# LLNL/ppo_and_friends

Hardware: AMD Instinct MI355X
Metric: env_steps_per_sec (higher is better)
Workload: dtype f32; 1 GPU; C2 CartPole-v1 MLP (4->128x3->2 actor, ->1 critic), envs_per_proc=4096, ts_per_rollout=128, fixed-length synthetic trajectories, batch_size=256, epochs_per_iter=10; parallelism=dp1, hip_graphs=True

## Files before the change

### ppo_and_friends_amd/csrc/ppo_update_dev.hpp

```cpp
#pragma once
#include "action_heads.hpp"
#include <cstddef>
#include <cstring>

namespace ppoaf {

struct WsDev {
    float* hbuf[2];
    float* dbuf[2];
    float* outpart[2];
    float* xbuf[2];
    int W;
    int xcc[2];
    int Bp;
};

struct UpdateDev {
    NetDev net[2];
    const float* params; float* grads; float* exp_avg; float* exp_avg_sq; float* slabs;
    long bucket_total;
    int64_t* step_counts; const float* lr; double* norm_scratch;
    float beta1, beta2, adam_eps, grad_scale, max_norm; int head_kind;
    const float* obs; const float* critic_obs; const void* raw_actions;
    const float* adv; const float* old_lp; const float* rtg; float* values;
    const int64_t* perm; const int32_t* row_map; long n_rows;
    int64_t* cursor; long B, batch_stride, mb_offset, cursor_advance;
    int normalize_values, n_ranks;
    float* vn_mean; float* vn_var; double* vn_count; const double* vn_records;
    const double* adv_records;
    int normalize_adv, use_huber, pregathered;
    float surr_clip, entropy_weight, kl_loss_weight, huber_delta, min_std;
    float* loss_partials; double* totals;
    int n_wg;
    int confine;
    int split;
    WsDev sp;
    int n_slices; int slices[8];
};

inline long ws_seg_off(const NetDev& n) {
    const long szW0 = ((long)n.H * n.in_dim + 3) & ~3L;
    return n.depth == 0 ? 0 : szW0 + n.H + (long)(n.depth - 1) * ((long)n.H * n.H + n.H);
}
inline long ws_seg_len(const NetDev& n) { return n.size - ws_seg_off(n); }

inline int split_wgrad_jobs(const NetDev& n) {
    const int t = n.H / 16, t2 = (t + 1) / 2, p0 = ((n.in_dim + 15) / 16 + 1) / 2;
    return (n.depth - 1) * t * t2 + t * p0 + 1;
}
inline int split_wgrad_per_xcd(const UpdateDev& u) { return (split_wgrad_jobs(u.net[0]) + split_wgrad_jobs(u.net[1]) + 7) / 8; }
inline int split_wgrad_blocks(const UpdateDev& u) { return 8 * split_wgrad_per_xcd(u); }

inline size_t ws_layout(const UpdateDev& u, WsDev* ws, char* base) {
    const long Bp = (u.B + 63) & ~63L;
    size_t off = 0;
    auto take = [&](size_t floats) { const size_t o = off; off += (floats * 4 + 255) & ~(size_t)255; return o; };
    for (int w = 0; w < 2; ++w) {
        const NetDev& n = u.net[w];
        const size_t plane = (size_t)n.depth * Bp * n.H;
        const size_t oh = take(plane), od = take(plane), oo = take((size_t)((u.B + 15) / 16) * ws_seg_len(n));
        const size_t ox = take((size_t)Bp * 64);
        if (ws) {
            ws->hbuf[w] = reinterpret_cast<float*>(base + oh);
            ws->dbuf[w] = reinterpret_cast<float*>(base + od);
            ws->outpart[w] = reinterpret_cast<float*>(base + oo);
            ws->xbuf[w] = reinterpret_cast<float*>(base + ox);
        }
    }
    if (ws) ws->Bp = (int)Bp;
    return off;
}

constexpr int kPairHeaderBytes = 256;
constexpr int kPairRecBytes = 16 * 1024;
constexpr int kPairMaxTiles = 32;
constexpr long long kPairWaitTicks = 200000000LL;

struct PairDev {
    unsigned char* base;
    long net_off[2];
};

inline bool pair_eligible(const NetDev& n) { return n.H == 256 && n.depth >= 2 && n.depth <= 4; }
inline int pair_phases(const NetDev& n) { return 2 * n.depth - 3; }
inline size_t pair_region_offset(const UpdateDev& u) {
    UpdateDev f = u;
    if (u.batch_stride > f.B) f.B = u.batch_stride;
    return ws_layout(f, nullptr, nullptr);
}
inline size_t pair_region_layout(const UpdateDev& u, PairDev* p, char* region) {
    size_t off = kPairHeaderBytes;
    for (int w = 0; w < 2; ++w) {
        const bool on = pair_eligible(u.net[w]);
        if (p) p->net_off[w] = on ? (long)off : 0;
        if (on) off += (size_t)pair_phases(u.net[w]) * kPairMaxTiles * 2 * kPairRecBytes;
    }
    if (p) p->base = reinterpret_cast<unsigned char*>(region);
    return off;
}

constexpr int kWgradThreads = 256;

__device__ __forceinline__ void ppo_update_bookkeeping_totals(const UpdateDev& u) {
    const int lane = threadIdx.x;
    float p0 = 0.f, p2 = 0.f, p3 = 0.f, p4 = 0.f, p7 = 0.f;
    for (int g = lane; g < u.n_wg; g += 64) {
        const float* a = u.loss_partials + (long)g * 8;
        const float* cc = u.loss_partials + ((long)u.n_wg + g) * 8;
        p0 += a[0]; p3 += a[3]; p4 += a[4]; p7 += a[7]; p2 += cc[2];
    }
    p0 = wave_sum(p0); p2 = wave_sum(p2); p3 = wave_sum(p3); p4 = wave_sum(p4); p7 = wave_sum(p7);
    if (lane == 0) {
        const float n = (float)u.B;
        const float surr = p0 / n, ent = p3 / n, kl = p4 / n, crit = p2 / n;
        float total = surr;
        if (u.entropy_weight != 0.0f) total -= u.entropy_weight * ent;
        if (u.kl_loss_weight > 0.0f) total += u.kl_loss_weight * kl;
        u.totals[0] += (double)surr; u.totals[1] += (double)total; u.totals[2] += (double)crit;
        u.totals[3] += (double)ent; u.totals[4] += (double)kl;
        u.totals[5] += (double)u.loss_partials[5]; u.totals[6] += (double)u.loss_partials[6];
        u.totals[7] += p7 > 0.f ? 1.0 : 0.0;
        u.totals[8] += 1.0;
    }
}
__device__ __forceinline__ void ppo_update_bookkeeping_steps(const UpdateDev& u) {
    const int lane = threadIdx.x;
    if (lane < 2) {
        const int w = lane;
        const int64_t t = u.step_counts[w] + 1;
        u.step_counts[w] = t;
        u.norm_scratch[2 + 2 * w] = 1.0 - pow((double)u.beta1, (double)t);
        u.norm_scratch[3 + 2 * w] = sqrt(1.0 - pow((double)u.beta2, (double)t));
    }
}

__device__ __forceinline__ void ppo_update_bookkeeping_split(const UpdateDev& u) {
    if (threadIdx.x >= 64) return;
    ppo_update_bookkeeping_totals(u);
    ppo_update_bookkeeping_steps(u);
}

int make_update_dev(const ppoaf_ppo_update_args_t* a, UpdateDev& u);

inline ppoaf_ppo_update_args_t copy_update_args(const ppoaf_ppo_update_args_t* args) {
    ppoaf_ppo_update_args_t a;
    std::memset(&a, 0, sizeof(a));
    std::memcpy(&a, args, offsetof(ppoaf_ppo_update_args_t, n_action_slices));
    if (args->head_kind == PPOAF_HEAD_MULTI_CATEGORICAL) {
        a.n_action_slices = args->n_action_slices;
        std::memcpy(a.action_slices, args->action_slices, sizeof(a.action_slices));
    }
    return a;
}

__device__ __forceinline__ unsigned hw_xcc_id() {
    unsigned v;
    asm volatile("s_getreg_b32 %0, hwreg(HW_REG_XCC_ID)" : "=s"(v));
    return v & 0xfu;
}

template <bool NT, typename U>
__device__ __forceinline__ void ppo_head_loss(const U& u, const int which, const int g, const int out_dim,
                                              const float* __restrict__ log_std_p, const int* sRow,
                                              const float* sRowF, const float* sMisc, float* sActF, float* sOut,
                                              float* sDOut, const int lane, const long B) {
    const int s = lane;
    const int row = s < kRows ? sRow[s] : -1;
    const bool live = row >= 0;
    const float inv_B = 1.0f / (float)B;
    float part[8] = {0, 0, 0, 0, 0, 0, 0, 0};
    if (which == 0) {
        float logp = 0.f, ent = 0.f;
        float av = 0.f, lpo = 0.f;
        if (live) {
            av = sRowF[s]; lpo = sRowF[16 + s];
            if (u.normalize_adv) av = (av - sMisc[0]) / (sMisc[1] + 1e-8f);
        }
        if (u.head_kind == PPOAF_HEAD_CATEGORICAL) {
            const int s4 = lane >> 2, q = lane & 3;
            const bool live4 = sRow[s4] >= 0;
            float av4 = 0.f, lpo4 = 0.f;
            if (live4) {
                av4 = sRowF[s4]; lpo4 = sRowF[16 + s4];
                if (u.normalize_adv) av4 = (av4 - sMisc[0]) / (sMisc[1] + 1e-8f);
            }
            auto rsum = [](float v) { return group4_sum(v); };
            auto rmax = [](float v) { return group4_max(v); };
            const int k0 = q, k1 = q + 4;
            const bool v0 = k0 < out_dim, v1 = k1 < out_dim;
            const float z0 = v0 ? sOut[s4 * kMaxOut + k0] : -INFINITY, z1 = v1 ? sOut[s4 * kMaxOut + k1] : -INFINITY;
            const float m = rmax(fmaxf(z0, z1));
            float p0 = v0 ? expf(z0 - m) : 0.f, p1 = v1 ? expf(z1 - m) : 0.f;
            const float inv = 1.0f / rsum(p0 + p1);
            p0 *= inv; p1 *= inv;
            const float s2 = rsum(p0 + p1);
            int a = reinterpret_cast<const int*>(sActF)[s4 * 8];
            a = a < 0 ? 0 : (a >= out_dim ? out_dim - 1 : a);
            const float n0 = p0 / s2, n1 = p1 / s2;
            const float l0 = v0 ? logf(clamp_prob_u(n0)) : 0.f, l1 = v1 ? logf(clamp_prob_u(n1)) : 0.f;
            const float ent4 = -rsum((v0 ? n0 * l0 : 0.f) + (v1 ? n1 * l1 : 0.f));
            const float logp4 = rsum((k0 == a ? l0 : 0.f) + (k1 == a ? l1 : 0.f));
            const float ratio = expf(logp4 - lpo4);
            const float bad4 = (isnan(ratio) || isinf(ratio)) ? 1.f : 0.f;
            const float lo = 1.0f - u.surr_clip, hi = 1.0f + u.surr_clip;
            const float surr1 = ratio * av4, surr2 = fminf(fmaxf(ratio, lo), hi) * av4;
            float glp;
            if (surr1 <= surr2) glp = -av4 * ratio;
            else glp = (ratio >= lo && ratio <= hi) ? -av4 * ratio : 0.f;
            glp *= inv_B;
            const float gH = (u.entropy_weight != 0.0f) ? -u.entropy_weight * inv_B : 0.f;
            auto gk_of = [&](bool valid, int k, float nk, float lg) {
                if (!valid) return 0.f;
                const float ck = clamp_prob_u(nk);
                const float in_range = (nk >= FLT_EPSILON && nk <= 1.0f - FLT_EPSILON) ? 1.f : 0.f;
                float gk = gH * (-lg - nk * in_range / ck);
                if (k == a) gk += glp * in_range / ck;
                return gk;
            };
            float g0 = gk_of(v0, k0, n0, l0), g1 = gk_of(v1, k1, n1, l1);
            const float dot = rsum(g0 * n0 + g1 * n1);
            g0 = (g0 - dot) / s2; g1 = (g1 - dot) / s2;
            const float dot2 = rsum(g0 * p0 + g1 * p1);
            if (live4) {
                if (k0 < 8) sDOut[s4 * kMaxOut + k0] = p0 * (g0 - dot2);
                sDOut[s4 * kMaxOut + k1] = p1 * (g1 - dot2);
            } else {
                sDOut[s4 * kMaxOut + k0] = 0.f; sDOut[s4 * kMaxOut + k1] = 0.f;
                if (q == 0) for (int k2 = 8; k2 < kMaxOut; ++k2) sDOut[s4 * kMaxOut + k2] = 0.f;
            }
            const int src = (lane & 15) * 4;
            const float r_surr = __shfl(-fminf(surr1, surr2), src, 64), r_ent = __shfl(ent4, src, 64);
            const float r_kl = __shfl(lpo4 - logp4, src, 64), r_bad = __shfl(bad4, src, 64);
            if (live) { part[0] = r_surr; part[3] = r_ent; part[4] = r_kl; part[7] = r_bad; }
        } else if (u.head_kind >= PPOAF_HEAD_MULTI_CATEGORICAL) {
            if (live) {
                float z[8], dz[8];
#pragma unroll
                for (int k = 0; k < 8; ++k) z[k] = k < out_dim ? sOut[s * kMaxOut + k] : 0.f;
                const bool mcat = u.head_kind == PPOAF_HEAD_MULTI_CATEGORICAL;
                const float* x = sActF + s * 8;
                float p[8], sm[8];
                unsigned first = 0u, pick = 0u;
                if (mcat) {
                    first = mcat_starts(u.n_slices, u.slices);
                    mcat_probs(z, first, out_dim, p, sm);
                    pick = mcat_pick(reinterpret_cast<const int*>(x), u.n_slices, u.slices);
                    logp = mcat_logp(p, sm, pick);
                } else {
                    logp = bern_logp(z, x, out_dim);
                }
                const float ratio = expf(logp - lpo);
                if (isnan(ratio) || isinf(ratio)) part[7] = 1.f;
                const float lo = 1.0f - u.surr_clip, hi = 1.0f + u.surr_clip;
                const float surr1 = ratio * av, surr2 = fminf(fmaxf(ratio, lo), hi) * av;
                float glp;
                if (surr1 <= surr2) glp = -av * ratio;
                else glp = (ratio >= lo && ratio <= hi) ? -av * ratio : 0.f;
                glp *= inv_B;
                const float gH = (u.entropy_weight != 0.0f) ? -u.entropy_weight * inv_B : 0.f;
                ent = mcat ? mcat_entropy_grad(p, sm, first, pick, out_dim, glp, gH, dz)
                           : bern_entropy_grad(z, x, out_dim, glp, gH, dz);
                part[0] = -fminf(surr1, surr2);
                part[3] = ent;
                part[4] = lpo - logp;
#pragma unroll
                for (int k = 0; k < 8; ++k) sDOut[s * kMaxOut + k] = dz[k];
            } else if (s < kRows) {
                for (int k = 0; k < kMaxOut; ++k) sDOut[s * kMaxOut + k] = 0.f;
            }
        } else if (live) {
            const float* log_std = log_std_p;
            const float* x = sActF + s * 8;
            float lp = 0.f, slog = 0.f;
            ent = 0.f;
            for (int d = 0; d < out_dim; ++d) {
                const float sd = fmaxf(softplus_u(ld1<NT>(log_std + d)), u.min_std);
                const float mu = sOut[s * kMaxOut + d];
                const float zz = x[d] - mu;
                const float l0 = -logf(sd) - 0.91893853320467274178f;
                float l = -(zz * zz) / (2.0f * sd * sd) + l0;
                l = fminf(fmaxf(l, -100.f), 100.f);
                lp += l;
                const float th = tanhf(x[d]);
                slog += logf(fmaxf(1.0f - th * th, 1e-6f));
                const float thm = tanhf(mu);
                ent += logf(fmaxf(1.0f - thm * thm, 1e-6f)) - fminf(fmaxf(l0, -100.f), 100.f);
            }
            logp = lp - slog;
            const float ratio = expf(logp - lpo);
            if (isnan(ratio) || isinf(ratio)) part[7] = 1.f;
            const float lo = 1.0f - u.surr_clip, hi = 1.0f + u.surr_clip;
            const float surr1 = ratio * av, surr2 = fminf(fmaxf(ratio, lo), hi) * av;
            part[0] = -fminf(surr1, surr2);
            part[3] = ent;
            part[4] = lpo - logp;
            float glp;
            if (surr1 <= surr2) glp = -av * ratio;
            else glp = (ratio >= lo && ratio <= hi) ? -av * ratio : 0.f;
            glp *= inv_B;
            const float gH = (u.entropy_weight != 0.0f) ? -u.entropy_weight * inv_B : 0.f;
            for (int d = 0; d < out_dim; ++d) {
                const float ls = ld1<NT>(log_std + d);
                const float sp = softplus_u(ls), sd = fmaxf(sp, u.min_std);
                const float mu = sOut[s * kMaxOut + d];
                const float zz = x[d] - mu;
                const float l0 = -logf(sd) - 0.91893853320467274178f;
                const float l = -(zz * zz) / (2.0f * sd * sd) + l0;
                const float pass = (l >= -100.f && l <= 100.f) ? 1.f : 0.f;
                const float pass0 = (l0 >= -100.f && l0 <= 100.f) ? 1.f : 0.f;
                const float thm = tanhf(mu);
                const float pass_t = (1.0f - thm * thm >= 1e-6f) ? 1.f : 0.f;
                sDOut[s * kMaxOut + d] = glp * pass * zz / (sd * sd) - gH * pass_t * 2.0f * thm;
                if (d == 0) for (int k2 = out_dim; k2 < 8; ++k2) sDOut[s * kMaxOut + k2] = 0.f;
                const float dmax = sp > u.min_std ? 1.f : (sp == u.min_std ? 0.5f : 0.f);
                const float dsp = ls > 20.f ? 1.f : 1.0f / (1.0f + expf(-ls));
                sOut[s * kMaxOut + 8 + d] = (glp * pass * (zz * zz / (sd * sd * sd) - 1.0f / sd) + gH * pass0 / sd) * dmax * dsp;
            }
        } else if (s < kRows) {
            for (int k = 0; k < kMaxOut; ++k) sDOut[s * kMaxOut + k] = 0.f;
            if (u.head_kind == PPOAF_HEAD_GAUSSIAN)
                for (int d = 0; d < 8; ++d) sOut[s * kMaxOut + 8 + d] = 0.f;
        }
    } else {
        if (live) {
            const float v = sOut[s * kMaxOut];
            float rt = sRowF[32 + s];
            if (u.normalize_values) rt = (rt - sMisc[2]) / sqrtf(sMisc[3] + 1e-8f);
            const float diff = v - rt;
            float l, dl;
            if (u.use_huber) {
                const float ad = fabsf(diff);
                if (ad < u.huber_delta) { l = 0.5f * diff * diff; dl = diff; }
                else { l = u.huber_delta * (ad - 0.5f * u.huber_delta); dl = diff > 0.f ? u.huber_delta : -u.huber_delta; }
            } else { l = diff * diff; dl = 2.0f * diff; }
            part[2] = l;
            sDOut[s * kMaxOut] = dl * inv_B;
            for (int k2 = 1; k2 < 8; ++k2) sDOut[s * kMaxOut + k2] = 0.f;
            u.values[row] = v;
        } else if (s < kRows) {
            for (int k2 = 0; k2 < 8; ++k2) sDOut[s * kMaxOut + k2] = 0.f;
        }
    }
#pragma unroll
    for (int k = 0; k < 8; ++k) {
        float v = (lane < kRows) ? part[k] : 0.f;
        v = group16_sum(v);
        part[k] = v;
    }
    if (lane == 0) {
        if (which == 0 && g == 0) { part[5] = sMisc[0]; part[6] = sMisc[1]; }
        float* lp = u.loss_partials + ((long)which * u.n_wg + g) * 8;
#pragma unroll
        for (int k = 0; k < 8; ++k) lp[k] = part[k];
    }
}

}
```

### ppo_and_friends_amd/csrc/ppo_update_rowtile.hpp

```cpp
#pragma once
#include "ppo_update_dev.hpp"

namespace ppoaf {

extern __shared__ __attribute__((aligned(16))) unsigned char ppo_update_smem[];

#ifdef PPOAF_STAMPS
#ifndef PPOAF_STAMP_BLOCK
#define PPOAF_STAMP_BLOCK 0
#endif
static __device__ unsigned long long g_ppo_update_stamps[2][16];
#define PPOAF_STAMP(k)                                                                   \
    do {                                                                                 \
        if (blockIdx.x == PPOAF_STAMP_BLOCK && threadIdx.x == 0) {                       \
            unsigned long long t_;                                                       \
            asm volatile("s_memtime %0\n\ts_waitcnt lgkmcnt(0)" : "=s"(t_)::"memory");    \
            g_ppo_update_stamps[0][k] = t_;                                              \
        }                                                                                \
    } while (0)
#else
#define PPOAF_STAMP(k) do {} while (0)
#endif



template <int HT, bool NT>
__device__ __forceinline__ void load_fwd_set(const float* __restrict__ W, int n0, int lane, float4 (&fr)[HT]) {
    if constexpr (NT) load_fwd_frags<HT, true>(W, n0, lane, fr);
    else load_fwd_lines_buf<HT>(W, n0, lane, fr);
}
template <int HT, bool NT>
__device__ __forceinline__ f32x4 mfma_fwd_set(const float* __restrict__ A, int HS, int lane, const float4 (&fr)[HT], float init,
                                              float* __restrict__ scratch) {
    if constexpr (NT) return mfma_rows_x_frags<HT>(A, HS, lane, fr, init);
    else return mfma_rows_x_lines<HT>(A, HS, lane, fr, init, scratch);
}

__device__ __forceinline__ int rowtile_request_args(const UpdateDev& u, int b) {
    const NetDev& a = u.net[0];
    const NetDev& c = u.net[1];
    asm("" : "+s"(b)
        : "s"(a.in_dim), "s"(a.H), "s"(a.depth), "s"(a.out_dim), "s"(a.act), "s"((&a.act)[1]), "s"(a.offset), "s"(a.size), "s"(a.log_std_off),
          "s"(c.in_dim), "s"(c.H), "s"(c.depth), "s"(c.out_dim), "s"(c.act), "s"((&c.act)[1]), "s"(c.offset), "s"(c.size), "s"(c.log_std_off),
          "s"(u.params), "s"(u.norm_scratch), "s"(u.head_kind),
          "s"(u.obs), "s"(u.critic_obs), "s"(u.raw_actions), "s"(u.adv), "s"(u.old_lp), "s"(u.rtg), "s"(u.values), "s"(u.perm),
          "s"(u.row_map), "s"(u.n_rows), "s"(u.cursor), "s"(u.B), "s"(u.batch_stride), "s"(u.mb_offset), "s"(u.cursor_advance),
          "s"(u.normalize_values), "s"(u.n_ranks), "s"(u.vn_mean), "s"(u.vn_var), "s"(u.vn_count), "s"(u.vn_records),
          "s"(u.adv_records), "s"(u.normalize_adv), "s"(u.use_huber), "s"(u.pregathered), "s"(u.surr_clip),
          "s"(u.n_wg), "s"(u.confine));
    const long cur = u.cursor[0];
    asm("" : "+s"(b)
        : "s"(cur), "s"(u.entropy_weight), "s"(u.kl_loss_weight), "s"(u.huber_delta), "s"(u.min_std), "s"(u.loss_partials),
          "s"(u.sp.hbuf[0]), "s"(u.sp.hbuf[1]), "s"(u.sp.dbuf[0]), "s"(u.sp.dbuf[1]), "s"(u.sp.outpart[0]), "s"(u.sp.outpart[1]),
          "s"(u.sp.xbuf[0]), "s"(u.sp.xbuf[1]), "s"(u.sp.W), "s"(u.sp.xcc[0]), "s"(u.sp.xcc[1]), "s"(u.sp.Bp), "s"(u.n_slices),
          "s"(u.slices[0]), "s"(u.slices[1]), "s"(u.slices[2]), "s"(u.slices[3]), "s"(u.slices[4]), "s"(u.slices[5]),
          "s"(u.slices[6]), "s"(u.slices[7]));
    return b;
}

template <int HT, bool SPLIT, bool TABLES>
__device__ __forceinline__ void ppo_update_fwd_bwd_body_as(const UpdateDev& u, const int which, const int g) {
    constexpr bool NT = false;
    constexpr long mb_extra = 0;
    constexpr int H = 16 * HT, HS = H + 4;
    int tid_ = threadIdx.x;
    if (NT) {
        asm volatile("" : "+v"(tid_));
        __builtin_assume(tid_ >= 0 && tid_ < kThreadsU);
    }
    const int tid = tid_, lane = tid & 63, wave = NT ? __builtin_amdgcn_readfirstlane(tid >> 6) : (tid >> 6);
    const auto& nd = u.net[which];
    const int in_dim = nd.in_dim, depth = nd.depth, out_dim = nd.out_dim, act = nd.act;
    const int NT0 = (in_dim + 15) >> 4;
    const int INP = 16 * NT0 + 4;
    const float* P = u.params + nd.offset;
    const long B = u.B;
    const long mb = u.cursor[0] + u.mb_offset + mb_extra;
    const long base = mb * u.batch_stride;
    const long szW0 = ((long)H * in_dim + 3) & ~3L;
    auto offW = [&](int l) -> long { return l == 0 ? 0 : szW0 + H + (long)(l - 1) * (H * H + H); };
    auto offB = [&](int l) -> long {
        return l == 0 ? szW0 : offW(l) + (l < depth ? (long)H * H : (((long)out_dim * H + 3) & ~3L));
    };
    float* slab = SPLIT ? u.sp.outpart[which] + (long)g * (nd.size - offW(depth)) - offW(depth)
                        : u.slabs + (long)g * u.bucket_total + nd.offset;
    auto publish_rows = [&](const float* src, float* panel) {
        float* dst = panel + (long)g * kRows * H;
        for (int i = tid; i < kRows * (H / 4); i += kThreadsU) {
            const int r = i / (H / 4), c4 = i - r * (H / 4);
            *reinterpret_cast<float4*>(dst + (long)r * H + 4 * c4) = *reinterpret_cast<const float4*>(src + r * HS + 4 * c4);
        }
    };
    const long sp_plane = SPLIT ? (long)u.sp.Bp * H : 0;

    PPOAF_STAMP(0);
    int zl = 0;
    if (NT) asm volatile("" : "+s"(zl));
    float* smem = reinterpret_cast<float*>(ppo_update_smem + zl);
    int* sRow = reinterpret_cast<int*>(smem);
    float* sMisc = smem + 16;
    float* sRowF = smem + 32;
    float* sActF = smem + 80;
    float* sBias = smem + 208;
    float* sWout = sBias + (depth + 1) * H;
    float* sX = sWout + 8 * H;
    float* sH = sX + kRows * INP;
    float* sD0 = sH + (long)depth * kRows * HS;
    float* sD1 = sD0 + kRows * HS;
    float* sOut = sD1 + kRows * HS;
    float* sDOut = sOut + kRows * kMaxOut;
    float* sScr = sDOut + kRows * kMaxOut + wave * 2 * kLineSlot;

    if (!NT && g == 0 && which == 0 && tid == 0) { u.norm_scratch[0] = 0.0; u.norm_scratch[1] = 0.0; }

    const bool has_tile = HT >= kNW || wave < HT;
    static_assert(!TABLES || HT <= kNW, "deep prefetch: one output tile per wave");
    const bool deep = TABLES || (depth == 3 && HT <= kNW);
    float4 fr[HT], fr2[HT];
    const bool l0_pre = in_dim <= 16 && HT <= kNW && has_tile;
    float l0w[4] = {0.f, 0.f, 0.f, 0.f};
    float l2_touch = 0.f;
    constexpr int kCopyRegs = 4;
    float bias_reg[kCopyRegs], wout_reg[kCopyRegs];
    const int n_bias = (depth + 1) * H, n_wout = out_dim * H;
    const bool copy_fits = n_bias <= kCopyRegs * kThreadsU && n_wout <= kCopyRegs * kThreadsU;
    auto request_weights = [&]() {
        if (NT && deep && has_tile) {
            load_fwd_set<HT, NT>(P + offW(1), wave * 16, lane, fr);
            load_fwd_set<HT, NT>(P + offW(2), wave * 16, lane, fr2);
        }
        if (l0_pre) {
            const float* w = P + offW(0) + (long)(wave * 16 + (lane & 15)) * in_dim;
#pragma unroll
            for (int j = 0; j < 4; ++j) { const int k = 4 * j + (lane >> 4); if (k < in_dim) l0w[j] = ld1<NT>(w + k); }
        }
#ifndef PPOAF_L2_TOUCH_MAX_HT
#define PPOAF_L2_TOUCH_MAX_HT 8
#endif
        if (!deep && !NT && HT <= PPOAF_L2_TOUCH_MAX_HT) for (long i = (long)tid * 32; i < nd.size; i += (long)kThreadsU * 32) l2_touch += P[i];
        if (copy_fits) {
#pragma unroll
            for (int r = 0; r < kCopyRegs; ++r) {
                const int i = tid + r * kThreadsU;
                bias_reg[r] = 0.f; wout_reg[r] = 0.f;
                if (i < n_bias) { const int l = i / H, j = i - l * H; if (l < depth || j < out_dim) bias_reg[r] = ld1<NT>(P + offB(l) + j); }
                if (i < n_wout) wout_reg[r] = ld1<NT>(P + offW(depth) + i);
            }
        }
    };
    auto request_hidden_sets = [&]() {
        if (!NT && deep && has_tile) {
            load_fwd_set<HT, NT>(P + offW(1), wave * 16, lane, fr);
            load_fwd_set<HT, NT>(P + offW(2), wave * 16, lane, fr2);
        }
    };
    const float* x_src = which == 0 ? u.obs : u.critic_obs;
    const bool x_pre = !NT && (TABLES || u.pregathered) && kRows * in_dim <= 2 * kThreadsU;
    float xr[2] = {0.f, 0.f};
    if (x_pre) {
#pragma unroll
        for (int q = 0; q < 2; ++q) {
            const int idx = tid + q * kThreadsU;
            if (idx < kRows * in_dim && (long)g * kRows + idx / in_dim < B) xr[q] = x_src[(base + (long)g * kRows) * in_dim + idx];
        }
    }
    if constexpr (TABLES) asm volatile("; ppoaf_rowtile_tables_prologue");
    if (!NT) request_weights();

    constexpr int kActRegs = 8;
    constexpr int kVnPre = 2;
    const bool row_lane = tid < kRows && (long)g * kRows + tid < B;
    static_assert(!TABLES || !NT, "per-epoch tables: separate launches only");
    constexpr bool early = TABLES;
    const int n_act = which != 0 ? 0 : u.head_kind == PPOAF_HEAD_CATEGORICAL ? 1
                    : u.head_kind == PPOAF_HEAD_MULTI_CATEGORICAL ? u.n_slices : out_dim;
    long perm_v = -1;
    float av = 0.f, lpo = 0.f, rt = 0.f;
    int act_bits[kActRegs];
#pragma unroll
    for (int j = 0; j < kActRegs; ++j) act_bits[j] = 0;
    auto request_row_scalars = [&](const long di) {
        if (which == 0) {
            av = u.adv[di]; lpo = u.old_lp[di];
            if (u.head_kind == PPOAF_HEAD_CATEGORICAL) {
                act_bits[0] = (int)reinterpret_cast<const int64_t*>(u.raw_actions)[di];
            } else if (u.head_kind == PPOAF_HEAD_MULTI_CATEGORICAL) {
#pragma unroll
                for (int j = 0; j < kActRegs; ++j)
                    if (j < n_act) act_bits[j] = (int)reinterpret_cast<const int64_t*>(u.raw_actions)[(long)di * u.n_slices + j];
            } else {
#pragma unroll
                for (int d = 0; d < kActRegs; ++d)
                    if (d < n_act) act_bits[d] = __float_as_int(reinterpret_cast<const float*>(u.raw_actions)[(long)di * out_dim + d]);
            }
        } else {
            rt = u.rtg[di];
        }
    };
    if (row_lane) {
        const long s = (long)g * kRows + tid;
        perm_v = u.perm[base + s];
        if (early) request_row_scalars(base + s);
    }
    const bool stat_lane = tid == 64;
    double adv_rec[3] = {0.0, 0.0, 0.0}, vn_rec[kVnPre][3];
    float vn_m = 0.f, vn_v = 0.f;
    double vn_cnt = 0.0;
#pragma unroll
    for (int r = 0; r < kVnPre; ++r) { vn_rec[r][0] = 0.0; vn_rec[r][1] = 0.0; vn_rec[r][2] = 0.0; }
    if (stat_lane) {
        if (which == 0) {
            if (u.normalize_adv) {
                const double* rec = u.adv_records + mb * 3;
                adv_rec[0] = rec[0]; adv_rec[1] = rec[1]; adv_rec[2] = rec[2];
            }
        } else {
            const int slot = (int)(mb & 1);
            vn_m = ld1<NT>(u.vn_mean + slot); vn_v = ld1<NT>(u.vn_var + slot);
            vn_cnt = ld1<NT>(u.vn_count + slot);
            if (u.normalize_values) {
#pragma unroll
                for (int r = 0; r < kVnPre; ++r) {
                    if (r < u.n_ranks) {
                        const double* rec = u.vn_records + (mb * u.n_ranks + r) * 3;
                        vn_rec[r][0] = rec[0]; vn_rec[r][1] = rec[1]; vn_rec[r][2] = rec[2];
                    }
                }
            }
        }
    }
    double vn_n = 0.0, vn_bm = 0.0, vn_M2 = 0.0;
    auto vn_merge = [&](const double nb, const double mean, const double m2) {
        if (nb <= 0.0) return;
        const double d = mean - vn_bm, nn = vn_n + nb;
        vn_bm += d * (nb / nn);
        vn_M2 += m2 + d * d * vn_n * nb / nn;
        vn_n = nn;
    };
    if (stat_lane && which != 0 && u.normalize_values && u.n_ranks > kVnPre) {
#pragma unroll
        for (int r = 0; r < kVnPre; ++r) vn_merge(vn_rec[r][0], vn_rec[r][1], vn_rec[r][2]);
        for (int r = kVnPre; r < u.n_ranks; ++r) {
            const double* rec = u.vn_records + (mb * u.n_ranks + r) * 3;
            vn_merge(rec[0], rec[1], rec[2]);
        }
    }
    if (!NT) request_hidden_sets();

    if (tid < kRows) {
        auto store_row = [&](const int row, const bool have) {
            if (have) {
#pragma unroll
                for (int j = 0; j < kActRegs; ++j)
                    if (j < n_act) reinterpret_cast<int*>(sActF)[tid * 8 + j] = act_bits[j];
            }
            sRow[tid] = row;
            sRowF[tid] = av; sRowF[16 + tid] = lpo; sRowF[32 + tid] = rt;
        };
        if constexpr (TABLES) {
            int row = -1;
            if (row_lane && perm_v >= 0 && perm_v < u.n_rows) row = (int)perm_v;
            store_row(row, row_lane);
        } else {
            int row = -1;
            long di = -1;
            if (row_lane) {
                const long p = perm_v;
                if (p >= 0 && p < u.n_rows) row = u.row_map ? u.row_map[p] : (int)p;
                di = u.pregathered ? base + (long)g * kRows + tid : row;
            }
            if (di >= 0 && !early) request_row_scalars(di);
            store_row(row, di >= 0);
        }
    }

    if (stat_lane) {
        if (which == 0) {
            float mean_f = 0.f, std_f = 1.f;
            if (u.normalize_adv) {
                mean_f = (float)adv_rec[1];
                std_f = (float)sqrt(adv_rec[2] / (adv_rec[0] - 1.0));
            }
            sMisc[0] = mean_f; sMisc[1] = std_f;
        } else {
            const int slot = (int)(mb & 1);
            float m = vn_m, v = vn_v;
            double cnt = vn_cnt;
            if (u.normalize_values) {
                if (u.n_ranks <= kVnPre) {
#pragma unroll
                    for (int r = 0; r < kVnPre; ++r)
                        if (r < u.n_ranks) vn_merge(vn_rec[r][0], vn_rec[r][1], vn_rec[r][2]);
                }
                const double n = vn_n, bm = vn_bm, M2 = vn_M2;
                if (n > 0.0) {
                    const float batch_mean = (float)bm, batch_var = (float)(M2 / n);
                    const float delta = batch_mean - m;
                    const double new_count = cnt + n;
                    const float new_mean = (float)((double)m + (double)delta * (n / new_count));
                    const double m_2 = (double)v * cnt + (double)batch_var * n +
                                       (double)(delta * delta) * cnt * n / (cnt + n);
                    m = new_mean; v = (float)(m_2 / (cnt + n)); cnt = new_count;
                }
            }
            sMisc[2] = m; sMisc[3] = v;
            if (g == 0) { u.vn_mean[slot ^ 1] = m; u.vn_var[slot ^ 1] = v; u.vn_count[slot ^ 1] = cnt; }
        }
    }
    if (copy_fits) {
#pragma unroll
        for (int r = 0; r < kCopyRegs; ++r) {
            const int i = tid + r * kThreadsU;
            if (i < n_bias) sBias[i] = bias_reg[r];
            if (i < n_wout) sWout[i] = wout_reg[r];
        }
    } else {
        for (int l = 0; l <= depth; ++l) {
            const int n = (l == depth) ? out_dim : H;
            const float* bb = P + offB(l);
            for (int i = tid; i < n; i += kThreadsU) sBias[l * H + i] = ld1<NT>(bb + i);
        }
        for (int i = tid; i < out_dim * H; i += kThreadsU) sWout[i] = ld1<NT>(P + offW(depth) + i);
    }
    for (int i = tid; i < kRows * INP; i += kThreadsU) sX[i] = 0.f;
    __syncthreads();
    PPOAF_STAMP(1);

    if (x_pre) {
#pragma unroll
        for (int q = 0; q < 2; ++q) {
            const int idx = tid + q * kThreadsU;
            const int s = idx / in_dim, i = idx - s * in_dim;
            if (idx < kRows * in_dim && sRow[s] >= 0) sX[s * INP + i] = xr[q];
        }
    } else {
        const float* src = x_src;
        for (int idx = tid; idx < kRows * in_dim; idx += kThreadsU) {
            const int s = idx / in_dim, i = idx - s * in_dim;
            const int row = sRow[s];
            const long di = (TABLES || u.pregathered) ? base + (long)g * kRows + s : row;
            if (row >= 0) sX[s * INP + i] = src[di * in_dim + i];
        }
    }
    if (!deep && depth > 1 && has_tile) load_fwd_set<HT, NT>(P + offW(1), wave * 16, lane, fr);
    __syncthreads();
    PPOAF_STAMP(2);
    if (SPLIT) {
        float* xb = u.sp.xbuf[which] + (long)g * kRows * 64;
        for (int i = tid; i < kRows * 64; i += kThreadsU) {
            const int r = i >> 6, c = i & 63;
            xb[i] = c < 16 * NT0 ? sX[r * INP + c] : 0.f;
        }
    }

    for (int nt = wave; nt < HT; nt += kNW) {
        const int o = nt * 16 + (lane & 15);
        const float bv = sBias[o];
        f32x4 acc = {bv, bv, bv, bv};
        const float* w = P + offW(0) + (long)o * in_dim;
        const float* arow = sX + (lane & 15) * INP;
        for (int k0 = 0; k0 < in_dim; k0 += 16) {
            float bq[4];
#pragma unroll
            for (int j = 0; j < 4; ++j) {
                const int k = k0 + 4 * j + (lane >> 4);
                bq[j] = l0_pre ? l0w[j] : (k < in_dim ? ld1<NT>(w + k) : 0.f);
            }
#pragma unroll
            for (int j = 0; j < 4; ++j)
                acc = __builtin_amdgcn_mfma_f32_16x16x4f32(arow[k0 + 4 * j + (lane >> 4)], bq[j], acc, 0, 0, 0);
        }
#pragma unroll
        for (int r = 0; r < 4; ++r) sH[(4 * (lane >> 4) + r) * HS + o] = act_fwd(acc[r], act);
    }
    __syncthreads();
    PPOAF_STAMP(3);

    for (int l = 1; l < depth; ++l) {
        const float* Hp = sH + (long)(l - 1) * kRows * HS;
        float* Hc = sH + (long)l * kRows * HS;
        if (SPLIT) publish_rows(Hp, u.sp.hbuf[which] + (long)(l - 1) * sp_plane);
        for (int nt = wave; nt < HT; nt += kNW) {
            const int o = nt * 16 + (lane & 15);
            f32x4 acc;
            if (deep) {
                if (l == 1) {
                    acc = mfma_fwd_set<HT, NT>(Hp, HS, lane, fr, sBias[l * H + o], sScr);
                    load_dgrad_frags<HT, NT>(P + offW(2), wave * 16, lane, fr);
                } else {
                    acc = mfma_fwd_set<HT, NT>(Hp, HS, lane, fr2, sBias[l * H + o], sScr);
                    load_dgrad_frags<HT, NT>(P + offW(1), wave * 16, lane, fr2);
                }
            } else {
            if (nt != wave) load_fwd_set<HT, NT>(P + offW(l), nt * 16, lane, fr);
            acc = mfma_fwd_set<HT, NT>(Hp, HS, lane, fr, sBias[l * H + o], sScr);
            if (nt + kNW >= HT) {
                if (l + 1 < depth) load_fwd_set<HT, NT>(P + offW(l + 1), wave * 16, lane, fr);
                else load_dgrad_frags<HT, NT>(P + offW(l), wave * 16, lane, fr);
            }
            }
#pragma unroll
            for (int r = 0; r < 4; ++r) Hc[(4 * (lane >> 4) + r) * HS + o] = act_fwd(acc[r], act);
            
        }
        __syncthreads();
        
    }
    PPOAF_STAMP(4);
    const float* Hlast = sH + (long)(depth - 1) * kRows * HS;

    if (tid < 256) {
        const int s = tid >> 4, part = tid & 15;
        for (int k = 0; k < out_dim; ++k) {
            float acc = 0.f;
#pragma unroll
            for (int i = 0; i < HT; ++i) acc = fmaf(Hlast[s * HS + part + 16 * i], sWout[k * H + part + 16 * i], acc);
            acc = group16_sum(acc);
            if (part == 0) sOut[s * kMaxOut + k] = acc + sBias[depth * H + k];
        }
    }
    __syncthreads();
    PPOAF_STAMP(5);

    if (wave == 0) {
        ppo_head_loss<NT>(u, which, g, out_dim, P + nd.log_std_off, sRow, sRowF, sMisc, sActF, sOut, sDOut, lane, B);
    }
    __syncthreads();
    PPOAF_STAMP(6);

    {
        if (tid < H) {
            const int i = tid;
            float h[kRows];
#pragma unroll
            for (int s = 0; s < kRows; ++s) h[s] = Hlast[s * HS + i];
            for (int k = 0; k < out_dim; ++k) {
                float d[kRows];
#pragma unroll
                for (int s = 0; s < kRows; ++s) d[s] = sDOut[s * kMaxOut + k];
                float acc = 0.f;
#pragma unroll
                for (int s = 0; s < kRows; ++s) acc = fmaf(d[s], h[s], acc);
                slab[offW(depth) + (long)k * H + i] = acc;
            }
        }
        const int out_pad = SPLIT ? ((out_dim + 3) & ~3) : out_dim;
        if (tid >= 256 && tid < 256 + out_pad) {
            const int k = tid - 256;
            float acc = 0.f;
            if (k < out_dim) {
#pragma unroll
                for (int s = 0; s < kRows; ++s) acc += sDOut[s * kMaxOut + k];
            }
            slab[offB(depth) + k] = acc;
        }
        if (which == 0 && u.head_kind == PPOAF_HEAD_GAUSSIAN && tid >= 320 && tid < 320 + out_pad) {
            const int d = tid - 320;
            float acc = 0.f;
            if (d < out_dim) {
#pragma unroll
                for (int s = 0; s < kRows; ++s) acc += sOut[s * kMaxOut + 8 + d];
            }
            slab[nd.log_std_off + d] = acc;
        }
        if (tid >= 256) {
            const int t2 = tid - 256;
            const int s = t2 >> 4, ig = t2 & 15;
            float d[8];
            const float4 d0 = *reinterpret_cast<const float4*>(sDOut + s * kMaxOut);
            const float4 d1 = *reinterpret_cast<const float4*>(sDOut + s * kMaxOut + 4);
            d[0] = d0.x; d[1] = d0.y; d[2] = d0.z; d[3] = d0.w; d[4] = d1.x; d[5] = d1.y; d[6] = d1.z; d[7] = d1.w;
            float hv[HT], acc[HT];
#pragma unroll
            for (int ii = 0; ii < HT; ++ii) { hv[ii] = Hlast[s * HS + ig + 16 * ii]; acc[ii] = 0.f; }
#pragma unroll
            for (int k = 0; k < 8; ++k) {
                if (k < out_dim) {
#pragma unroll
                    for (int ii = 0; ii < HT; ++ii) acc[ii] = fmaf(d[k], sWout[k * H + ig + 16 * ii], acc[ii]);
                }
            }
#pragma unroll
            for (int ii = 0; ii < HT; ++ii) sD0[s * HS + ig + 16 * ii] = acc[ii] * act_bwd(hv[ii], act);
        }
    }
    __syncthreads();
    PPOAF_STAMP(7);

    float* Dc = sD0;
    float* Dn = sD1;
    for (int l = depth - 1; l >= 1; --l) {
        const float* Hin = sH + (long)(l - 1) * kRows * HS;
        if (SPLIT) publish_rows(Dc, u.sp.dbuf[which] + (long)l * sp_plane);
        for (int nt = wave; nt < HT; nt += kNW) {
            f32x4 acc;
            if (deep) {
                acc = l == 2 ? mfma_rows_x_frags<HT>(Dc, HS, lane, fr, 0.f) : mfma_rows_x_frags<HT>(Dc, HS, lane, fr2, 0.f);
            } else {
            if (nt != wave) load_dgrad_frags<HT, NT>(P + offW(l), nt * 16, lane, fr);
            acc = mfma_rows_x_frags<HT>(Dc, HS, lane, fr, 0.f);
            if (nt + kNW >= HT && l - 1 >= 1) load_dgrad_frags<HT, NT>(P + offW(l - 1), wave * 16, lane, fr);
            }
#pragma unroll
            for (int r = 0; r < 4; ++r) {
                const int s = 4 * (lane >> 4) + r, i = nt * 16 + (lane & 15);
                Dn[s * HS + i] = acc[r] * act_bwd(Hin[s * HS + i], act);
            }
        }
        if (l == depth - 1) PPOAF_STAMP(10);
        if (!SPLIT) {
            for (int mt = wave; mt < HT; mt += kNW) {
                if (HT <= 8) wgrad_mtile_full<(HT <= 8 ? HT : 1)>(Dc, HS, Hin, HS, mt * 16, lane, slab + offW(l), H);
                else wgrad_mtile(Dc, HS, Hin, HS, mt * 16, HT, H, lane, slab + offW(l), H);
            }
            if (l == depth - 1) PPOAF_STAMP(11);
            for (int o = tid; o < H; o += kThreadsU) {
                float acc = 0.f;
#pragma unroll
                for (int s = 0; s < kRows; ++s) acc += Dc[s * HS + o];
                slab[offB(l) + o] = acc;
            }
        }
        if (l == depth - 1) PPOAF_STAMP(12);
        __syncthreads();
        if (l == depth - 1) PPOAF_STAMP(13);
        float* t = Dc; Dc = Dn; Dn = t;
    }
    PPOAF_STAMP(8);

    if (SPLIT) {
        publish_rows(Dc, u.sp.dbuf[which]);
    } else {
        for (int mt = wave; mt < HT; mt += kNW)
            wgrad_mtile(Dc, HS, sX, INP, mt * 16, NT0, in_dim, lane, slab + offW(0), in_dim);
        for (int o = tid; o < H; o += kThreadsU) {
            float acc = 0.f;
#pragma unroll
            for (int s = 0; s < kRows; ++s) acc += Dc[s * HS + o];
            slab[offB(0) + o] = acc;
        }
    }
    if (l2_touch == 1.2345e38f) u.loss_partials[0] = l2_touch;
    PPOAF_STAMP(9);
}

template <int HT, bool SPLIT = false>
__device__ __forceinline__ void ppo_update_fwd_bwd_body(const UpdateDev& u, const int which, const int g) {
    if constexpr (HT <= kNW) {
        if (u.net[which].depth == 3 && u.pregathered && !u.row_map) {
            ppo_update_fwd_bwd_body_as<HT, SPLIT, true>(u, which, g);
            return;
        }
    }
    ppo_update_fwd_bwd_body_as<HT, SPLIT, false>(u, which, g);
}

constexpr size_t kRowtileLineFloats = (size_t)kNW * 2 * kLineSlot;
inline size_t rowtile_lds_floats(const NetDev& n) {
    const size_t HS = n.H + 4, INP = 16 * ((n.in_dim + 15) / 16) + 4;
    return 208 + (size_t)(n.depth + 1) * n.H + 8 * (size_t)n.H + kRows * INP + (size_t)n.depth * kRows * HS + 2 * kRows * HS +
           2 * kRows * kMaxOut;
}

}
```

Before: 1.133 million env-steps/s.

## Fuse head forward, loss and dgrad per row-group and defer head weight-grad tail

In the TABLES path, each 16-lane group now computes its row's output logits, head loss and output dgrad itself, separated only by wavefront barriers, so two block-wide __syncthreads are gone. The head loss is split into a per-row function, and the loss-partial reduction, output weight-grad and bias grads move into a deferred tail. By default that tail runs inside the first hidden backward layer, overlapping with the MFMA dgrad work. The change also keeps the first two output-weight rows in registers and preloads the Hlast column for the tail threads, which raises register pressure.

After: 1.133 million env-steps/s, median of 2. No clear change (+0.0%).

```diff
diff --git a/ppo_and_friends_amd/csrc/ppo_update_dev.hpp b/ppo_and_friends_amd/csrc/ppo_update_dev.hpp
--- a/ppo_and_friends_amd/csrc/ppo_update_dev.hpp
+++ b/ppo_and_friends_amd/csrc/ppo_update_dev.hpp
@@ -159,16 +159,14 @@
     return v & 0xfu;
 }
 
-template <bool NT, typename U>
-__device__ __forceinline__ void ppo_head_loss(const U& u, const int which, const int g, const int out_dim,
-                                              const float* __restrict__ log_std_p, const int* sRow,
-                                              const float* sRowF, const float* sMisc, float* sActF, float* sOut,
-                                              float* sDOut, const int lane, const long B) {
-    const int s = lane;
-    const int row = s < kRows ? sRow[s] : -1;
+template <bool NT, typename U, typename Z>
+__device__ __forceinline__ void ppo_head_row(const U& u, const int which, const int out_dim,
+                                             const float* __restrict__ log_std_p, const int* sRow, const float* sRowF,
+                                             const float* sMisc, const float* sActF, float* sOut, float* sDOut, const int s,
+                                             const int q, const bool writer, const Z& zval, const long B, float (&part)[8]) {
+    const int row = sRow[s];
     const bool live = row >= 0;
     const float inv_B = 1.0f / (float)B;
-    float part[8] = {0, 0, 0, 0, 0, 0, 0, 0};
     if (which == 0) {
         float logp = 0.f, ent = 0.f;
         float av = 0.f, lpo = 0.f;
@@ -177,36 +175,29 @@
             if (u.normalize_adv) av = (av - sMisc[0]) / (sMisc[1] + 1e-8f);
         }
         if (u.head_kind == PPOAF_HEAD_CATEGORICAL) {
-            const int s4 = lane >> 2, q = lane & 3;
-            const bool live4 = sRow[s4] >= 0;
-            float av4 = 0.f, lpo4 = 0.f;
-            if (live4) {
-                av4 = sRowF[s4]; lpo4 = sRowF[16 + s4];
-                if (u.normalize_adv) av4 = (av4 - sMisc[0]) / (sMisc[1] + 1e-8f);
-            }
             auto rsum = [](float v) { return group4_sum(v); };
             auto rmax = [](float v) { return group4_max(v); };
             const int k0 = q, k1 = q + 4;
             const bool v0 = k0 < out_dim, v1 = k1 < out_dim;
-            const float z0 = v0 ? sOut[s4 * kMaxOut + k0] : -INFINITY, z1 = v1 ? sOut[s4 * kMaxOut + k1] : -INFINITY;
+            const float z0 = v0 ? zval(k0) : -INFINITY, z1 = v1 ? zval(k1) : -INFINITY;
             const float m = rmax(fmaxf(z0, z1));
             float p0 = v0 ? expf(z0 - m) : 0.f, p1 = v1 ? expf(z1 - m) : 0.f;
             const float inv = 1.0f / rsum(p0 + p1);
             p0 *= inv; p1 *= inv;
             const float s2 = rsum(p0 + p1);
-            int a = reinterpret_cast<const int*>(sActF)[s4 * 8];
+            int a = reinterpret_cast<const int*>(sActF)[s * 8];
             a = a < 0 ? 0 : (a >= out_dim ? out_dim - 1 : a);
             const float n0 = p0 / s2, n1 = p1 / s2;
             const float l0 = v0 ? logf(clamp_prob_u(n0)) : 0.f, l1 = v1 ? logf(clamp_prob_u(n1)) : 0.f;
             const float ent4 = -rsum((v0 ? n0 * l0 : 0.f) + (v1 ? n1 * l1 : 0.f));
             const float logp4 = rsum((k0 == a ? l0 : 0.f) + (k1 == a ? l1 : 0.f));
-            const float ratio = expf(logp4 - lpo4);
+            const float ratio = expf(logp4 - lpo);
             const float bad4 = (isnan(ratio) || isinf(ratio)) ? 1.f : 0.f;
             const float lo = 1.0f - u.surr_clip, hi = 1.0f + u.surr_clip;
-            const float surr1 = ratio * av4, surr2 = fminf(fmaxf(ratio, lo), hi) * av4;
+            const float surr1 = ratio * av, surr2 = fminf(fmaxf(ratio, lo), hi) * av;
             float glp;
-            if (surr1 <= surr2) glp = -av4 * ratio;
-            else glp = (ratio >= lo && ratio <= hi) ? -av4 * ratio : 0.f;
+            if (surr1 <= surr2) glp = -av * ratio;
+            else glp = (ratio >= lo && ratio <= hi) ? -av * ratio : 0.f;
             glp *= inv_B;
             const float gH = (u.entropy_weight != 0.0f) ? -u.entropy_weight * inv_B : 0.f;
             auto gk_of = [&](bool valid, int k, float nk, float lg) {
@@ -221,22 +212,21 @@
             const float dot = rsum(g0 * n0 + g1 * n1);
             g0 = (g0 - dot) / s2; g1 = (g1 - dot) / s2;
             const float dot2 = rsum(g0 * p0 + g1 * p1);
-            if (live4) {
-                if (k0 < 8) sDOut[s4 * kMaxOut + k0] = p0 * (g0 - dot2);
-                sDOut[s4 * kMaxOut + k1] = p1 * (g1 - dot2);
-            } else {
-                sDOut[s4 * kMaxOut + k0] = 0.f; sDOut[s4 * kMaxOut + k1] = 0.f;
-                if (q == 0) for (int k2 = 8; k2 < kMaxOut; ++k2) sDOut[s4 * kMaxOut + k2] = 0.f;
+            if (writer) {
+                if (live) {
+                    if (k0 < 8) sDOut[s * kMaxOut + k0] = p0 * (g0 - dot2);
+                    sDOut[s * kMaxOut + k1] = p1 * (g1 - dot2);
+                } else {
+                    sDOut[s * kMaxOut + k0] = 0.f; sDOut[s * kMaxOut + k1] = 0.f;
+                    if (q == 0) for (int k2 = 8; k2 < kMaxOut; ++k2) sDOut[s * kMaxOut + k2] = 0.f;
+                }
             }
-            const int src = (lane & 15) * 4;
-            const float r_surr = __shfl(-fminf(surr1, surr2), src, 64), r_ent = __shfl(ent4, src, 64);
-            const float r_kl = __shfl(lpo4 - logp4, src, 64), r_bad = __shfl(bad4, src, 64);
-            if (live) { part[0] = r_surr; part[3] = r_ent; part[4] = r_kl; part[7] = r_bad; }
+            if (live) { part[0] = -fminf(surr1, surr2); part[3] = ent4; part[4] = lpo - logp4; part[7] = bad4; }
         } else if (u.head_kind >= PPOAF_HEAD_MULTI_CATEGORICAL) {
             if (live) {
                 float z[8], dz[8];
 #pragma unroll
-                for (int k = 0; k < 8; ++k) z[k] = k < out_dim ? sOut[s * kMaxOut + k] : 0.f;
+                for (int k = 0; k < 8; ++k) z[k] = k < out_dim ? zval(k) : 0.f;
                 const bool mcat = u.head_kind == PPOAF_HEAD_MULTI_CATEGORICAL;
                 const float* x = sActF + s * 8;
                 float p[8], sm[8];
@@ -265,7 +255,7 @@
                 part[4] = lpo - logp;
 #pragma unroll
                 for (int k = 0; k < 8; ++k) sDOut[s * kMaxOut + k] = dz[k];
-            } else if (s < kRows) {
+            } else {
                 for (int k = 0; k < kMaxOut; ++k) sDOut[s * kMaxOut + k] = 0.f;
             }
         } else if (live) {
@@ -275,7 +265,7 @@
             ent = 0.f;
             for (int d = 0; d < out_dim; ++d) {
                 const float sd = fmaxf(softplus_u(ld1<NT>(log_std + d)), u.min_std);
-                const float mu = sOut[s * kMaxOut + d];
+                const float mu = zval(d);
                 const float zz = x[d] - mu;
                 const float l0 = -logf(sd) - 0.91893853320467274178f;
                 float l = -(zz * zz) / (2.0f * sd * sd) + l0;
@@ -302,7 +292,7 @@
             for (int d = 0; d < out_dim; ++d) {
                 const float ls = ld1<NT>(log_std + d);
                 const float sp = softplus_u(ls), sd = fmaxf(sp, u.min_std);
-                const float mu = sOut[s * kMaxOut + d];
+                const float mu = zval(d);
                 const float zz = x[d] - mu;
                 const float l0 = -logf(sd) - 0.91893853320467274178f;
                 const float l = -(zz * zz) / (2.0f * sd * sd) + l0;
@@ -316,14 +306,14 @@
                 const float dsp = ls > 20.f ? 1.f : 1.0f / (1.0f + expf(-ls));
                 sOut[s * kMaxOut + 8 + d] = (glp * pass * (zz * zz / (sd * sd * sd) - 1.0f / sd) + gH * pass0 / sd) * dmax * dsp;
             }
-        } else if (s < kRows) {
+        } else {
             for (int k = 0; k < kMaxOut; ++k) sDOut[s * kMaxOut + k] = 0.f;
             if (u.head_kind == PPOAF_HEAD_GAUSSIAN)
                 for (int d = 0; d < 8; ++d) sOut[s * kMaxOut + 8 + d] = 0.f;
         }
     } else {
         if (live) {
-            const float v = sOut[s * kMaxOut];
+            const float v = zval(0);
             float rt = sRowF[32 + s];
             if (u.normalize_values) rt = (rt - sMisc[2]) / sqrtf(sMisc[3] + 1e-8f);
             const float diff = v - rt;
@@ -337,10 +327,15 @@
             sDOut[s * kMaxOut] = dl * inv_B;
             for (int k2 = 1; k2 < 8; ++k2) sDOut[s * kMaxOut + k2] = 0.f;
             u.values[row] = v;
-        } else if (s < kRows) {
+        } else {
             for (int k2 = 0; k2 < 8; ++k2) sDOut[s * kMaxOut + k2] = 0.f;
         }
     }
+}
+
+template <typename U>
+__device__ __forceinline__ void ppo_head_partials(const U& u, const int which, const int g, const float* sMisc,
+                                                  const int lane, float (&part)[8]) {
 #pragma unroll
     for (int k = 0; k < 8; ++k) {
         float v = (lane < kRows) ? part[k] : 0.f;
@@ -355,4 +350,25 @@
     }
 }
 
-}
+template <bool NT, typename U>
+__device__ __forceinline__ void ppo_head_loss(const U& u, const int which, const int g, const int out_dim,
+                                              const float* __restrict__ log_std_p, const int* sRow,
+                                              const float* sRowF, const float* sMisc, float* sActF, float* sOut,
+                                              float* sDOut, const int lane, const long B) {
+    float part[8] = {0, 0, 0, 0, 0, 0, 0, 0};
+    if (which == 0 && u.head_kind == PPOAF_HEAD_CATEGORICAL) {
+        const int s4 = lane >> 2;
+        float r[8] = {0, 0, 0, 0, 0, 0, 0, 0};
+        ppo_head_row<NT>(u, which, out_dim, log_std_p, sRow, sRowF, sMisc, sActF, sOut, sDOut, s4, lane & 3, true,
+                         [&](const int k) { return sOut[s4 * kMaxOut + k]; }, B, r);
+        const int src = (lane & 15) * 4;
+        part[0] = __shfl(r[0], src, 64); part[3] = __shfl(r[3], src, 64);
+        part[4] = __shfl(r[4], src, 64); part[7] = __shfl(r[7], src, 64);
+    } else if (lane < kRows) {
+        ppo_head_row<NT>(u, which, out_dim, log_std_p, sRow, sRowF, sMisc, sActF, sOut, sDOut, lane, 0, true,
+                         [&](const int k) { return sOut[lane * kMaxOut + k]; }, B, part);
+    }
+    ppo_head_partials(u, which, g, sMisc, lane, part);
+}
+
+}
diff --git a/ppo_and_friends_amd/csrc/ppo_update_rowtile.hpp b/ppo_and_friends_amd/csrc/ppo_update_rowtile.hpp
--- a/ppo_and_friends_amd/csrc/ppo_update_rowtile.hpp
+++ b/ppo_and_friends_amd/csrc/ppo_update_rowtile.hpp
@@ -409,83 +409,204 @@
     PPOAF_STAMP(4);
     const float* Hlast = sH + (long)(depth - 1) * kRows * HS;
 
-    if (tid < 256) {
-        const int s = tid >> 4, part = tid & 15;
-        for (int k = 0; k < out_dim; ++k) {
-            float acc = 0.f;
-#pragma unroll
-            for (int i = 0; i < HT; ++i) acc = fmaf(Hlast[s * HS + part + 16 * i], sWout[k * H + part + 16 * i], acc);
-            acc = group16_sum(acc);
-            if (part == 0) sOut[s * kMaxOut + k] = acc + sBias[depth * H + k];
-        }
-    }
-    __syncthreads();
-    PPOAF_STAMP(5);
-
-    if (wave == 0) {
-        ppo_head_loss<NT>(u, which, g, out_dim, P + nd.log_std_off, sRow, sRowF, sMisc, sActF, sOut, sDOut, lane, B);
-    }
-    __syncthreads();
-    PPOAF_STAMP(6);
-
-    {
-        if (tid < H) {
-            const int i = tid;
-            float h[kRows];
-#pragma unroll
-            for (int s = 0; s < kRows; ++s) h[s] = Hlast[s * HS + i];
-            for (int k = 0; k < out_dim; ++k) {
+    const int out_pad = SPLIT ? ((out_dim + 3) & ~3) : out_dim;
+#ifndef PPOAF_HEAD_TAIL_AT
+#define PPOAF_HEAD_TAIL_AT 1
+#endif
+    constexpr int kDwThreads = kThreadsU - 256;
+    constexpr bool kPreH = TABLES && PPOAF_HEAD_TAIL_AT != 2 && kDwThreads % H == 0;
+    float hcol[kRows];
+    auto head_tail = [&]() {
+        if (wave >= 4) {
+            for (int idx = tid - 256; idx < out_dim * H; idx += kDwThreads) {
+                const int k = idx / H, i = idx - k * H;
+                if (!kPreH) {
+#pragma unroll
+                    for (int s = 0; s < kRows; ++s) hcol[s] = Hlast[s * HS + i];
+                }
                 float d[kRows];
 #pragma unroll
                 for (int s = 0; s < kRows; ++s) d[s] = sDOut[s * kMaxOut + k];
                 float acc = 0.f;
 #pragma unroll
-                for (int s = 0; s < kRows; ++s) acc = fmaf(d[s], h[s], acc);
+                for (int s = 0; s < kRows; ++s) acc = fmaf(d[s], hcol[s], acc);
                 slab[offW(depth) + (long)k * H + i] = acc;
             }
-        }
-        const int out_pad = SPLIT ? ((out_dim + 3) & ~3) : out_dim;
-        if (tid >= 256 && tid < 256 + out_pad) {
-            const int k = tid - 256;
-            float acc = 0.f;
-            if (k < out_dim) {
-#pragma unroll
-                for (int s = 0; s < kRows; ++s) acc += sDOut[s * kMaxOut + k];
-            }
-            slab[offB(depth) + k] = acc;
-        }
-        if (which == 0 && u.head_kind == PPOAF_HEAD_GAUSSIAN && tid >= 320 && tid < 320 + out_pad) {
-            const int d = tid - 320;
-            float acc = 0.f;
-            if (d < out_dim) {
-#pragma unroll
-                for (int s = 0; s < kRows; ++s) acc += sOut[s * kMaxOut + 8 + d];
-            }
-            slab[nd.log_std_off + d] = acc;
-        }
-        if (tid >= 256) {
-            const int t2 = tid - 256;
-            const int s = t2 >> 4, ig = t2 & 15;
+        } else if (wave == 0) {
+            float part[8];
+#pragma unroll
+            for (int k = 0; k < 8; ++k) part[k] = lane < kRows ? sOut[lane * kMaxOut + k] : 0.f;
+            ppo_head_partials(u, which, g, sMisc, lane, part);
+        } else if (wave == 1) {
+            if (lane < out_pad) {
+                const int k = lane;
+                float acc = 0.f;
+                if (k < out_dim) {
+#pragma unroll
+                    for (int s = 0; s < kRows; ++s) acc += sDOut[s * kMaxOut + k];
+                }
+                slab[offB(depth) + k] = acc;
+            }
+        } else if (wave == 2) {
+            if (which == 0 && u.head_kind == PPOAF_HEAD_GAUSSIAN && lane < out_pad) {
+                const int d = lane;
+                float acc = 0.f;
+                if (d < out_dim) {
+#pragma unroll
+                    for (int s = 0; s < kRows; ++s) acc += sOut[s * kMaxOut + 8 + d];
+                }
+                slab[nd.log_std_off + d] = acc;
+            }
+        }
+    };
+    if constexpr (TABLES) {
+        asm volatile("; ppoaf_rowtile_head_phase_begin");
+        if (tid < 256) {
+            const int s = tid >> 4, part = tid & 15;
+            constexpr int kKeepW = 2;
+            float hv[HT], wk[kKeepW][HT];
+#pragma unroll
+            for (int i = 0; i < HT; ++i) { hv[i] = Hlast[s * HS + part + 16 * i]; wk[0][i] = 0.f; wk[1][i] = 0.f; }
+#pragma unroll
+            for (int k = 0; k < 8; ++k) {
+                if (k < out_dim) {
+                    float w[HT];
+#pragma unroll
+                    for (int i = 0; i < HT; ++i) w[i] = sWout[k * H + part + 16 * i];
+                    float acc = 0.f;
+#pragma unroll
+                    for (int i = 0; i < HT; ++i) acc = fmaf(hv[i], w[i], acc);
+                    if (k < kKeepW) {
+#pragma unroll
+                        for (int i = 0; i < HT; ++i) wk[k < kKeepW ? k : 0][i] = w[i];
+                    }
+                    acc = group16_sum(acc);
+                    if (part == 0) sOut[s * kMaxOut + k] = acc + sBias[depth * H + k];
+                }
+            }
+            __builtin_amdgcn_fence(__ATOMIC_ACQ_REL, "wavefront");
+            __builtin_amdgcn_wave_barrier();
+            PPOAF_STAMP(5);
+            auto zval = [&](const int k) { return sOut[s * kMaxOut + k]; };
+            float pr[8] = {0, 0, 0, 0, 0, 0, 0, 0};
+            if (which == 0 && u.head_kind == PPOAF_HEAD_CATEGORICAL) {
+                ppo_head_row<NT>(u, which, out_dim, P + nd.log_std_off, sRow, sRowF, sMisc, sActF, sOut, sDOut, s, part & 3,
+                                 part < 4, zval, B, pr);
+            } else if (part == 0) {
+                ppo_head_row<NT>(u, which, out_dim, P + nd.log_std_off, sRow, sRowF, sMisc, sActF, sOut, sDOut, s, 0, true,
+                                 zval, B, pr);
+            }
+            if (part == 0) {
+                *reinterpret_cast<float4*>(sOut + s * kMaxOut) = make_float4(pr[0], pr[1], pr[2], pr[3]);
+                *reinterpret_cast<float4*>(sOut + s * kMaxOut + 4) = make_float4(pr[4], pr[5], pr[6], pr[7]);
+            }
+            __builtin_amdgcn_fence(__ATOMIC_ACQ_REL, "wavefront");
+            __builtin_amdgcn_wave_barrier();
             float d[8];
             const float4 d0 = *reinterpret_cast<const float4*>(sDOut + s * kMaxOut);
             const float4 d1 = *reinterpret_cast<const float4*>(sDOut + s * kMaxOut + 4);
             d[0] = d0.x; d[1] = d0.y; d[2] = d0.z; d[3] = d0.w; d[4] = d1.x; d[5] = d1.y; d[6] = d1.z; d[7] = d1.w;
-            float hv[HT], acc[HT];
-#pragma unroll
-            for (int ii = 0; ii < HT; ++ii) { hv[ii] = Hlast[s * HS + ig + 16 * ii]; acc[ii] = 0.f; }
+            PPOAF_STAMP(6);
+            float acc[HT];
+#pragma unroll
+            for (int ii = 0; ii < HT; ++ii) acc[ii] = 0.f;
 #pragma unroll
             for (int k = 0; k < 8; ++k) {
                 if (k < out_dim) {
 #pragma unroll
-                    for (int ii = 0; ii < HT; ++ii) acc[ii] = fmaf(d[k], sWout[k * H + ig + 16 * ii], acc[ii]);
-                }
-            }
-#pragma unroll
-            for (int ii = 0; ii < HT; ++ii) sD0[s * HS + ig + 16 * ii] = acc[ii] * act_bwd(hv[ii], act);
-        }
-    }
-    __syncthreads();
-    PPOAF_STAMP(7);
+                    for (int ii = 0; ii < HT; ++ii)
+                        acc[ii] = fmaf(d[k], k < kKeepW ? wk[k < kKeepW ? k : 0][ii] : sWout[k * H + part + 16 * ii], acc[ii]);
+                }
+            }
+#pragma unroll
+            for (int ii = 0; ii < HT; ++ii) sD0[s * HS + part + 16 * ii] = acc[ii] * act_bwd(hv[ii], act);
+        } else if (kPreH) {
+            const int i = (tid - 256) % H;
+#pragma unroll
+            for (int s = 0; s < kRows; ++s) hcol[s] = Hlast[s * HS + i];
+        }
+        __syncthreads();
+        PPOAF_STAMP(7);
+        asm volatile("; ppoaf_rowtile_head_phase_end");
+        if (PPOAF_HEAD_TAIL_AT == 0) head_tail();
+    } else {
+        if (tid < 256) {
+            const int s = tid >> 4, part = tid & 15;
+            for (int k = 0; k < out_dim; ++k) {
+                float acc = 0.f;
+#pragma unroll
+                for (int i = 0; i < HT; ++i) acc = fmaf(Hlast[s * HS + part + 16 * i], sWout[k * H + part + 16 * i], acc);
+                acc = group16_sum(acc);
+                if (part == 0) sOut[s * kMaxOut + k] = acc + sBias[depth * H + k];
+            }
+        }
+        __syncthreads();
+        PPOAF_STAMP(5);
+
+        if (wave == 0) {
+            ppo_head_loss<NT>(u, which, g, out_dim, P + nd.log_std_off, sRow, sRowF, sMisc, sActF, sOut, sDOut, lane, B);
+        }
+        __syncthreads();
+        PPOAF_STAMP(6);
+
+        {
+            if (tid < H) {
+                const int i = tid;
+                float h[kRows];
+#pragma unroll
+                for (int s = 0; s < kRows; ++s) h[s] = Hlast[s * HS + i];
+                for (int k = 0; k < out_dim; ++k) {
+                    float d[kRows];
+#pragma unroll
+                    for (int s = 0; s < kRows; ++s) d[s] = sDOut[s * kMaxOut + k];
+                    float acc = 0.f;
+#pragma unroll
+                    for (int s = 0; s < kRows; ++s) acc = fmaf(d[s], h[s], acc);
+                    slab[offW(depth) + (long)k * H + i] = acc;
+                }
+            }
+            if (tid >= 256 && tid < 256 + out_pad) {
+                const int k = tid - 256;
+                float acc = 0.f;
+                if (k < out_dim) {
+#pragma unroll
+                    for (int s = 0; s < kRows; ++s) acc += sDOut[s * kMaxOut + k];
+                }
+                slab[offB(depth) + k] = acc;
+            }
+            if (which == 0 && u.head_kind == PPOAF_HEAD_GAUSSIAN && tid >= 320 && tid < 320 + out_pad) {
+                const int d = tid - 320;
+                float acc = 0.f;
+                if (d < out_dim) {
+#pragma unroll
+                    for (int s = 0; s < kRows; ++s) acc += sOut[s * kMaxOut + 8 + d];
+                }
+                slab[nd.log_std_off + d] = acc;
+            }
+            if (tid >= 256) {
+                const int t2 = tid - 256;
+                const int s = t2 >> 4, ig = t2 & 15;
+                float d[8];
+                const float4 d0 = *reinterpret_cast<const float4*>(sDOut + s * kMaxOut);
+                const float4 d1 = *reinterpret_cast<const float4*>(sDOut + s * kMaxOut + 4);
+                d[0] = d0.x; d[1] = d0.y; d[2] = d0.z; d[3] = d0.w; d[4] = d1.x; d[5] = d1.y; d[6] = d1.z; d[7] = d1.w;
+                float hv[HT], acc[HT];
+#pragma unroll
+                for (int ii = 0; ii < HT; ++ii) { hv[ii] = Hlast[s * HS + ig + 16 * ii]; acc[ii] = 0.f; }
+#pragma unroll
+                for (int k = 0; k < 8; ++k) {
+                    if (k < out_dim) {
+#pragma unroll
+                        for (int ii = 0; ii < HT; ++ii) acc[ii] = fmaf(d[k], sWout[k * H + ig + 16 * ii], acc[ii]);
+                    }
+                }
+#pragma unroll
+                for (int ii = 0; ii < HT; ++ii) sD0[s * HS + ig + 16 * ii] = acc[ii] * act_bwd(hv[ii], act);
+            }
+        }
+        __syncthreads();
+        PPOAF_STAMP(7);
+    }
 
     float* Dc = sD0;
     float* Dn = sD1;
@@ -508,6 +629,7 @@
             }
         }
         if (l == depth - 1) PPOAF_STAMP(10);
+        if constexpr (TABLES && PPOAF_HEAD_TAIL_AT == 1) { if (l == depth - 1) head_tail(); }
         if (!SPLIT) {
             for (int mt = wave; mt < HT; mt += kNW) {
                 if (HT <= 8) wgrad_mtile_full<(HT <= 8 ? HT : 1)>(Dc, HS, Hin, HS, mt * 16, lane, slab + offW(l), H);
@@ -540,6 +662,7 @@
             slab[offB(0) + o] = acc;
         }
     }
+    if constexpr (TABLES && PPOAF_HEAD_TAIL_AT == 2) head_tail();
     if (l2_touch == 1.2345e38f) u.loss_partials[0] = l2_touch;
     PPOAF_STAMP(9);
 }
```
